# iris1997jiatong/I-DCCRN-VAE

Measured on AMD Instinct MI355X. Metric: 4s@16kHz utterances/sec fwd+SI-SNR, DCCRN-CL, 1/2/4/8 MI355X vs host CPU, higher is better.
Workload: dtype f32; 1 GPU; supervised DCCRN-CL forward(train=False) + final_ete_loss (weights 0/0/1); batch_per_gpu=64, utterance=4 s @ 16 kHz (64000 samples, 641 frames), parallelism=replicas x1, streams=1, input=resident in HBM

## Files before the change

### i-dccrn-vae_amd/csrc/ctconv_c1_f32.hip

```cpp
#include "cgemm.hpp"
#include "conv_epilogue.hpp"
#include "../../include/idccrn_hip.h"

namespace {

constexpr int C1F_NC = 4;
constexpr int C1F_PR = 4;

template <bool STATS>
__global__ __launch_bounds__(256) void ctconv_c1_f32_kernel(const CgemmArgs a, int rseg) {
    const int tid = threadIdx.x;
    const int m_lo = blockIdx.y * rseg;
    int m_hi = m_lo + rseg;
    if (m_hi > a.Fin) m_hi = a.Fin;
    int jcol[C1F_NC], c0[C1F_NC][2], c1[C1F_NC][2];
    bool inb[C1F_NC], keep[C1F_NC], cok[C1F_NC][2];
#pragma unroll
    for (int n = 0; n < C1F_NC; ++n) {
        const int j = (blockIdx.x * C1F_NC + n) * 256 + tid;
        jcol[n] = j;
        inb[n] = j < a.J;
#pragma unroll
        for (int h = 0; h < 2; ++h) {
            const int c = j + h + a.tshift;
            cok[n][h] = inb[n] && c >= 0 && c < a.J;
            c0[n][h] = cok[n][h] ? c : 0;
            const int b = c0[n][h] / a.Tp;
            c1[n][h] = (b / a.x1_div) * a.Tp + (c0[n][h] - b * a.Tp);
        }
        const int tp = j % a.Tp;
        keep[n] = inb[n] && tp >= 1 && tp <= a.t_valid;
    }
    const float slope = a.slope ? *a.slope : 1.0f;
    const bool has_act = a.slope != nullptr;
    const float bias0 = a.bias[0], bias1 = a.bias[1];
    const size_t plane0 = (size_t)a.Fin * a.Jp, plane1 = (size_t)a.Fin * a.Jp1;
    const int CC = 2 * (a.C0 + a.C1);

    float st[5] = {0.f, 0.f, 0.f, 0.f, 0.f};
    float pa[C1F_NC][10], pb[C1F_NC][10], pc[C1F_NC][10];
#pragma unroll
    for (int n = 0; n < C1F_NC; ++n)
#pragma unroll
        for (int i = 0; i < 10; ++i) pa[n][i] = pb[n][i] = pc[n][i] = 0.f;

    auto contract = [&](int m, float (&p)[C1F_NC][10]) {
#pragma unroll
        for (int n = 0; n < C1F_NC; ++n)
#pragma unroll
            for (int i = 0; i < 10; ++i) p[n][i] = 0.f;
        if (m < 0 || m >= a.Fin) return;
        for (int cc0 = 0; cc0 < CC; cc0 += C1F_PR) {
            float xv[C1F_PR][C1F_NC][2];
#pragma unroll
            for (int u = 0; u < C1F_PR; ++u) {
                const int cc = cc0 + u < CC ? cc0 + u : CC - 1;
                const int ci = cc >> 1, ri = cc & 1;
                const bool first = ci < a.C0;
                const float* r = first ? a.x0 + (size_t)(ri * a.C0 + ci) * plane0 + (size_t)m * a.Jp
                                       : a.x1 + (size_t)(ri * a.C1 + (ci - a.C0)) * plane1 + (size_t)m * a.Jp1;
#pragma unroll
                for (int n = 0; n < C1F_NC; ++n) {
                    xv[u][n][0] = r[first ? c0[n][0] : c1[n][0]];
                    xv[u][n][1] = r[first ? c0[n][1] : c1[n][1]];
                }
            }
#pragma unroll
            for (int u = 0; u < C1F_PR; ++u) {
                const bool live = cc0 + u < CC;
                const float* w = a.wfrag + (size_t)(live ? cc0 + u : 0) * 5 * 64;
#pragma unroll
                for (int kf = 0; kf < 5; ++kf) {
                    const float w00 = live ? w[kf * 64] : 0.f, w01 = live ? w[kf * 64 + 1] : 0.f;
                    const float w10 = live ? w[kf * 64 + 32] : 0.f, w11 = live ? w[kf * 64 + 33] : 0.f;
#pragma unroll
                    for (int n = 0; n < C1F_NC; ++n) {
                        const float x0v = cok[n][0] ? xv[u][n][0] : 0.f, x1v = cok[n][1] ? xv[u][n][1] : 0.f;
                        p[n][kf * 2] += w00 * x0v;
                        p[n][kf * 2 + 1] += w01 * x0v;
                        p[n][kf * 2] += w10 * x1v;
                        p[n][kf * 2 + 1] += w11 * x1v;
                    }
                }
            }
        }
    };
    auto emit = [&](int n, int fo, float yr, float yi) {
        if (fo < 0 || fo >= a.Fout) return;
        yr += bias0;
        yi += bias1;
        if (has_act) {
            yr = yr >= 0.f ? yr : slope * yr;
            yi = yi >= 0.f ? yi : slope * yi;
        }
        yr = keep[n] ? yr : 0.f;
        yi = keep[n] ? yi : 0.f;
        if (inb[n]) {
            a.out[(size_t)fo * a.Jp + jcol[n]] = yr;
            a.out[((size_t)a.Fout + fo) * a.Jp + jcol[n]] = yi;
        }
        if (STATS && keep[n]) epi_stats_add(st, yr, yi);
    };

    contract(m_lo - 1, pa);
    contract(m_lo, pb);
    for (int m = m_lo; m < m_hi; ++m) {
        contract(m + 1, pc);
#pragma unroll
        for (int n = 0; n < C1F_NC; ++n) {
            emit(n, 2 * m, pc[n][0] + pb[n][4] + pa[n][8], pc[n][1] + pb[n][5] + pa[n][9]);
            emit(n, 2 * m + 1, pc[n][2] + pb[n][6], pc[n][3] + pb[n][7]);
#pragma unroll
            for (int i = 0; i < 10; ++i) {
                pa[n][i] = pb[n][i];
                pb[n][i] = pc[n][i];
            }
        }
    }
    if (STATS) {
        __shared__ float red[4][5];
        const int lane = tid & 63, wave = tid >> 6;
#pragma unroll
        for (int s = 0; s < 5; ++s) {
            float t = st[s];
#pragma unroll
            for (int o = 32; o > 0; o >>= 1) t += __shfl_xor(t, o, 64);
            if (lane == 0) red[wave][s] = t;
        }
        __syncthreads();
        if (tid < 5) atomicAdd(&a.stats[tid], (double)red[0][tid] + (double)red[1][tid] + (double)red[2][tid] + (double)red[3][tid]);
    }
}

}

int idv_launch_ctconv_c1_f32(const CgemmArgs& a, hipStream_t st) {
    const int colblocks = (a.J + 256 * C1F_NC - 1) / (256 * C1F_NC);
    int segs = 512 / colblocks;
    if (segs < 1) segs = 1;
    if (segs > a.Fin) segs = a.Fin;
    const int rseg = (a.Fin + segs - 1) / segs;
    dim3 grid((unsigned)colblocks, (unsigned)((a.Fin + rseg - 1) / rseg));
    if (a.stats)
        hipLaunchKernelGGL(ctconv_c1_f32_kernel<true>, grid, dim3(256), 0, st, a, rseg);
    else
        hipLaunchKernelGGL(ctconv_c1_f32_kernel<false>, grid, dim3(256), 0, st, a, rseg);
    return idv_launch_status();
}
```

### include/idccrn_hip.h

```cpp
#ifndef IDCCRN_HIP_H
#define IDCCRN_HIP_H

#ifdef __cplusplus
extern "C" {
#endif

#define IDV_ABI_VERSION 9
#define IDV_SLACK_FLOATS 256

int idv_abi_version(void);

int idv_coop_last_status(int clear);
int idv_coop_max_workgroups(void);


int idv_cconv_cck(int cin_used);
int idv_cconv_config(int transposed, int cin_used, int Cout, int Fin);

int idv_cbn_fold(const float* moments, const float* gamma_rr, const float* gamma_ri, const float* gamma_ii,
                 const float* beta_r, const float* beta_i, int C, float* fold, void* stream);

int idv_pack_cconv(const float* w_re, const float* w_im, const float* b_re, const float* b_im, const float* fold,
                   int Cout, int Cin_total, int Cin_used, int transposed, float* wfrag, float* bias_out, void* stream);

int idv_pack_pw(const float* w, const float* bias, int M, int K, float* wfrag, float* bias_out, void* stream);

int idv_pack_lstm_ih(const float* w_ih_re, const float* b_ih_re, const float* b_hh_re, const float* w_ih_im,
                     const float* b_ih_im, const float* b_hh_im, int H, int K, float* wfrag, float* bias_out,
                     void* stream);
int idv_pack_lstm_hh(const float* w_hh_re, const float* w_hh_im, int H, float* whh_frag, void* stream);

int idv_make_dft(int n_fft, int win, int hop, int T, float* w_fwd, float* w_inv, float* env_inv, void* stream);


int idv_cconv2d_fwd(const float* x0, int C0, const float* x1, int C1, int Jp1, int x1_div, const float* wfrag,
                    const float* bias, const float* prelu_slope, float* out, double* stats, double* stats_work, int stats_rep,
                    int transposed, int tshift, int Cout, int Fin, int B, int Tp, int Jp, int t_valid_out, void* stream);

int idv_cconv_gauss_supported(int C0, int C1, int Cout);
long long idv_cconv_gauss_wfrag_floats(int Cout, int cin_used);
int idv_cconv_gauss_epi_rows(int Cout);
int idv_cconv_gauss_config(int transposed, int Cin, int Cout, int Fin);
int idv_pack_cconv_gauss(const float* w_re, const float* w_im, const float* b_re, const float* b_im, const float* fold, int Cout,
                         int Cin_total, int Cin_used, int transposed, int conj, float* wfrag, float* epi, void* stream);
int idv_cconv2d_gauss_fwd(const float* x0, int C0, const float* x1, int C1, int Jp1, int x1_div, const float* wfrag,
                          const float* epi, int has_fold, const float* prelu_slope, float* out, double* stats, double* stats_work,
                          int stats_rep, int transposed, int tshift, int Cout, int Fin, int B, int Tp, int Jp, int t_valid_out,
                          const float* addend, int addend_div, int addend_Jp, void* stream);

long long idv_cconv_bf16_wfrag_bytes(int Cout, int cin_used);
int idv_cconv_bf16_supported(int transposed, int C0, int C1, int x1_div, int Cout);
int idv_cconv_bf16_config(int transposed, int Cout, int Fin);
int idv_pack_cconv_bf16(const float* w_re, const float* w_im, const float* fold, int Cout, int Cin_total, int Cin_used,
                        int transposed, void* wfrag, void* stream);
int idv_cconv2d_bf16x3_fwd(const float* x0, int C0, const float* x1, int C1, int Jp1, int x1_div, const void* wfrag_bf16,
                           const float* bias, const float* prelu_slope, float* out, double* stats, double* stats_work,
                           int stats_rep, int transposed, int tshift, int Cout, int Fin, int B, int Tp, int Jp, int t_valid_out,
                           void* stream);

int idv_cconv2d_fwd_img(const float* x0, int C0, const float* x1, int C1, int Jp1, const float* wfrag, const float* bias,
                        const float* prelu_slope, float* out_planar, void* out_img, long long out_lo_off_elems,
                        int transposed, int tshift, int Cout, int Fin, int B, int Tp, int Jp, int t_valid_out,
                        void* stream);
int idv_cconv2d_img_train_fwd(const void* x0_img, long long lo_off0, int C0, const void* x1_img, long long lo_off1, int C1,
                              const void* wfrag_bf16, const float* bias, float* out_planar, double* stats, double* stats_work,
                              int stats_rep, int transposed, int Cout, int Fin, int B, int Tp, int Jp, int t_valid_out, void* stream);
int idv_cconv_img_config(int src_is_image, int transposed, int Cin, int Cout, int Fin);
int idv_planar_to_image(const float* x, int C, int F, int J, int Jp, void* img, long long lo_off_elems, void* stream);
int idv_planar_to_image_repeat(const float* x, int C, int F, int B, int Tp, int Jp_in, int rep, void* img, long long lo_off_elems,
                               int Jp, void* stream);
int idv_image_to_planar(const void* img, long long lo_off_elems, int C, int F, int J, int Jp, float* x, void* stream);
int idv_cconv2d_img_fwd(int src_is_image , const void* x0_img, long long lo_off0_slots, int C0, const void* x1_img, long long lo_off1_slots,
                        int C1, const void* wfrag_bf16, const float* bias, const float* prelu_slope, float* out_planar,
                        void* out_img, long long out_lo_off_elems, int transposed, int tshift,
                        int Cout, int Fin, int B, int Tp, int Jp, int t_valid_out, void* stream);

long long idv_ctconv_c1_wfrag_bytes(int cin_used);
int idv_pack_ctconv_c1_bf16(const float* w_re, const float* w_im, const float* fold, int Cin_total, int Cin_used,
                            void* wfrag, void* stream);
int idv_ctconv_c1_bf16x3_fwd(const float* x0, int C0, const float* x1, int C1, int Jp1, const void* wfrag,
                             const float* bias, const float* prelu_slope, float* out, int Fin, int B, int Tp, int Jp,
                             int t_valid_out, void* stream);
int idv_ctconv_c1_img_fwd(const void* x0_img, long long lo_off0_slots, int C0, const void* x1_img, long long lo_off1_slots,
                          int C1, const void* wfrag, const float* bias, const float* prelu_slope, float* out, int Fin, int B,
                          int Tp, int Jp, int t_valid_out, void* stream);

int idv_pw_gemm(const float* x, int K, const float* wfrag, const float* bias, const float* prelu_slope, float* out,
                int M, int B, int Tp, int Jp, int t_valid, int swap, int ldo, void* stream);
int idv_pw_gemm_form(int M, int swap, int Jp, const float* x);

int idv_cbn_finalize(const double* stats, double count, const float* gamma_rr, const float* gamma_ri,
                     const float* gamma_ii, const float* beta_r, const float* beta_i, int C, int first_call,
                     float momentum, float* running_mean_r, float* running_mean_i, float* Vrr, float* Vri,
                     float* Vii, float* moments, float* fold, void* stream);
int idv_cbn_stats(const float* act, int C, int F, int B, int Tp, int Jp, int t_valid, double* stats, void* stream);
int idv_cbn_apply_prelu(float* act, const float* fold, const float* prelu_slope, int C, int F, int B, int Tp, int Jp,
                        int t_valid, void* stream);

int idv_stft_frames(const float* x, int B, int L, int n_fft, int win, int hop, int T, float* frames, int Tp, int Jp,
                    void* stream);
int idv_istft_ola(const float* frames, const float* env_inv, int B, int n_fft, int win, int hop, int T, int Tp,
                  int Jp, float* y, void* stream);

int idv_mask_apply(const float* mask, const float* X, int x_div, int JpX, float* pred, float* pred_c, int F, int B,
                   int T, int Tp, int Jp, void* stream);
int idv_datanorm(const float* X, const float* mean, const float* stdv, int F, int B, int T, int Tp, int Jp, float* out, void* stream);
int idv_datadenorm(const float* P, const float* mean, const float* stdv, int F, int B, int T, int Tp, int Jp, float* out,
                   float* out_c, void* stream);
int idv_datanorm_bwd(const float* dout, const float* stdv, int F, int B, int T, int Tp, int Jp, float* dX, void* stream);
int idv_datadenorm_bwd(const float* dout, const float* dout_c, const float* stdv, int F, int B, int T, int Tp, int Jp, float* dP,
                       void* stream);
int idv_outtype_estimate(const float* speech_c, const float* noise_c, const float* X, long long sb, long long sf, long long st,
                         long long sr, int mode, int ns, int B, int F, int T, int Tp, int Jp, float* out, float* out_c,
                         void* stream);
int idv_planar_to_complex(const float* act, float* out_c, int F, int B, int T, int Tp, int Jp, void* stream);

long long idv_clstm_work_floats(int H, int B, int T, int Jp);
int idv_lstm_pers_supported(int H, int B);
long long idv_lstm_pers_work_bytes(int H, int B);
int idv_lstm_rec_pers(const float* g, long long g_run_z, long long g_run_s, int ldg, const float* whh_frag, float* hout, int H,
                      int B, int T, void* work, void* kimg, long long kimg_lo_slots, int Tp, int Jp, float* gsave, float* csave,
                      void* stream);
int idv_lstm_proj1_bf16x3(const void* himg, long long lo_off_slots, const void* wfrag_bf16, const float* bias, float* G1, int H,
                          int B, int T, int Tp, int Jp, void* stream);
int idv_lstm_coop_f32_supported(int H, int B);
long long idv_lstm_coop_f32_work_bytes(int H, int B);
int idv_lstm_rec_coop_f32(const float* g, long long g_run_z, long long g_run_s, int ldg, const float* whh_frag, float* hout, int H,
                          int B, int T, void* work, float* gsave, float* csave, void* stream);
int idv_lstm_pers_f32_supported(int H, int B);
long long idv_lstm_pers_f32_work_bytes(int H, int B);
int idv_lstm_rec_pers_f32(const float* g, long long g_run_z, long long g_run_s, int ldg, const float* whh_frag, float* hout, int H,
                          int B, int T, void* work, float* gsave, float* csave, void* stream);
void idv_lstm_pers_set_profile(unsigned long long* prof_cycles);
long long idv_clstm_train_work_floats(int H, int B, int T, int Jp);
int idv_clstm_fwd(const float* x, int K, const float* wih0, const float* bih0, const float* whh0, const float* wih1,
                  const float* bih1, const float* whh1, int H, int B, int T, int Tp, int Jp, float* work, float* out,
                  int flags, const void* wih1_bf16, void* stream);

int idv_lstm_stack2_f32_supported(int H, int B);
long long idv_lstm_stack2_f32_work_bytes(int H, int B);
int idv_lstm_stack2_f32(const float* g, long long g_run_z, long long g_run_s, int ldg, const float* whh0, const float* wih1_hh,
                        const float* whh1, const float* bias1, float* h0, float* hout, int H, int B, int T, void* work,
                        float* gsave1, float* csave0, float* csave1, void* stream);
int idv_clstm_fwd2(const float* x, int K, const float* wih0, const float* bih0, const float* whh0, const float* wih1,
                   const float* bih1, const float* whh1, const float* wih1_hh, int H, int B, int T, int Tp, int Jp, float* work,
                   float* out, int flags, const void* wih1_bf16, void* stream);

int idv_lstm_stack2_f32_proj_split(int H, int B, int T, int K, int force_c0, int* c0, int* P);
long long idv_lstm_stack2_f32_proj_work_bytes(int H, int B, int Tmax);
int idv_lstm_stack2_f32_proj(const float* x, int K, int Tp, int Jp, const float* wih0, const float* bih0, float* g,
                             const float* whh0, const float* wih1_hh, const float* whh1, const float* bias1, float* h0,
                             float* hout, int H, int B, int T, void* work, float* gsave1, float* csave0, float* csave1,
                             int force_c0, void* stream);
int idv_clstm_fwd3(const float* x, int K, const float* wih0, const float* bih0, const float* whh0, const float* wih1,
                   const float* bih1, const float* whh1, const float* wih1_hh, int H, int B, int T, int Tp, int Jp, float* work,
                   float* out, int flags, const void* wih1_bf16, int proj_c0, void* stream);

long long idv_lstm_ih_bf16_bytes(int H, int K);
int idv_lstm_proj_bf16_supported(int H, int K);
int idv_pack_lstm_ih_bf16(const float* w_ih_re, const float* w_ih_im, int H, int K, void* wfrag, void* stream);
int idv_planar_to_kimage(const float* x, int nvalid, int nplanes, int J, int Jp, void* img, long long lo_off_elems, void* stream);
int idv_pw_bf16_coltile(int M, int B, int Tp);
int idv_pw_bf16x3_rows(const void* ximg, long long lo_off_slots, int K, const void* wfrag_bf16, const float* bias, float* out_rows,
                       int M, int ldo, int B, int T, int Tp, int Jp, void* stream);
long long idv_pw_bf16_wfrag_bytes(int M, int K);
int idv_pack_pw_bf16(const float* w, int M, int K, void* wfrag, void* stream);
int idv_pw_bf16x3(const void* ximg, long long lo_off_slots, int K, const void* wfrag_bf16, const float* bias, float* out, int M,
                  int B, int Tp, int Jp, int t_valid, void* stream);
int idv_stft_frames_kimage(const float* x, int B, int L, int n_fft, int win, int hop, int T, void* img, long long lo_off_elems,
                           int Tp, int Jp, void* stream);
int idv_lstm_proj_bf16x3(const void* ximg, long long lo_off_slots, int K, const void* wfrag_bf16, const float* bias, float* G,
                         int H, int B, int T, int Tp, int Jp, void* stream);

int idv_reparam(const float* lat, int Hl, int off_miu, int off_ls, int off_dl, int zdim, const float* eps_r,
                const float* eps_i, int ns, int B, int T, int Tp, int Jp, float* z, int Jpz, void* stream);


int idv_sisnr(const float* source, int src_ld, int src_div, const float* est, int est_ld, int B, int L, double* work,
              float* out, void* stream);
int idv_sisdr(const float* ref, int ref_ld, const float* est, int est_ld, int B, int L, double* work, float* out, void* stream);
int idv_mean_over_samples(const float* x, int ns, int B, int L, float* out, void* stream);
int idv_recon_loss(const float* pred_c, const float* ori, long long sb, long long sf, long long st, long long sr,
                   int ori_div, int B, int F, int T, double* work, float* out, void* stream);
int idv_ckl(const float* q1, int H1, int Jp1, int o1_miu, int o1_ls, int o1_dl, const float* q2, int H2, int Jp2,
            int o2_miu, int o2_ls, int o2_dl, int zdim, float eps, int B, int T, int Tp, double* work, float* out,
            void* stream);
int idv_msd(const float* a, int Ca, int ca0, int JpA, const float* b, int Cb, int cb0, int JpB, int C, int F, int B, int Tp,
            int t_valid, double* work, float* out, void* stream);
long long idv_mi_work_floats(int B, int ns, int T, int zdim);
int idv_mi_fwd(const float* lat, int H, int Jp, int o_miu, int o_ls, int o_dl, const float* z, int Jpz, int zdim, int ns, int B,
               int T, int Tp, float eps, float* work, double* acc, float* out, void* stream);
int idv_mi_bwd(const float* lat, int H, int Jp, int o_miu, int o_ls, int o_dl, const float* z, int Jpz, int zdim, int ns, int B,
               int T, int Tp, float eps, const float* work, const float* gout, float* dlat, float* dz, void* stream);
int idv_miu_dist(const float* q1, int H1, int Jp1, int off1, const float* q2, int H2, int Jp2, int off2, int zdim,
                 int B, int T, int Tp, double* work, float* out, void* stream);


int idv_pack_cconv_adjoint(const float* w_re, const float* w_im, int Cout, int Cin_total, int Cin_used, int transposed,
                           float* wfrag, float* bias_out, void* stream);
int idv_pack_cconv_bf16_adjoint(const float* w_re, const float* w_im, int Cout, int Cin_total, int Cin_used, int transposed,
                                void* wfrag, void* stream);

long long idv_cconv_wgrad_work_floats(int Cs, int Cl, int B, int Tp);
int idv_cconv2d_bwd_weight(const float* x, int Cx, int ci_off, const float* dy, int Cout, int Cin_total, int transposed,
                           int tshift, int Fin, int B, int Tp, int Jp_x, int Jp_dy, float* work, long long work_floats,
                           float* dw_re, float* dw_im, void* stream);
long long idv_cconv_wgrad_bf16_work_floats(int Cs, int Cl, int B, int Tp);
int idv_cconv2d_bwd_weight_bf16x3(const float* x, int Cx, int ci_off, const float* dy, int Cout, int Cin_total, int transposed,
                                  int tshift, int Fin, int B, int Tp, int Jp_x, int Jp_dy, float* work, long long work_floats,
                                  float* dw_re, float* dw_im, void* stream);
int idv_cconv_wgrad_gauss_supported(int Cs, int Cl);
long long idv_cconv_wgrad_gauss_work_floats(int Cx, int Cout, int transposed, int Fin, int B, int Tp, int Jp_x, int Jp_dy);
int idv_cconv2d_bwd_weight_gauss(const float* x, int Cx, int ci_off, const float* dy, int Cout, int Cin_total, int transposed,
                                 int tshift, int Fin, int B, int Tp, int Jp_x, int Jp_dy, float* work, long long work_floats,
                                 float* dw_re, float* dw_im, void* stream);
int idv_cconv2d_bwd_bias(const double* stats_dy, int Cout, float* db_re, float* db_im, void* stream);

long long idv_pw_wgrad_work_floats(int M, int K, int J);
int idv_pw_bwd_weight(const float* dout, int M, int Jp_d, const float* x, int K, int Jp_x, int J, int shift, float* work,
                      long long work_floats, float* dw, int ldw, int rowmap, int H, int accumulate, void* stream);
int idv_pw_bwd_weight_bf16x3(const float* dout, int M, int Jp_d, const float* x, int K, int Jp_x, int J, int shift, float* work,
                             long long work_floats, float* dw, int ldw, int rowmap, int H, int accumulate, void* stream);
int idv_planar_rowsum(const float* x, int M, int Jp, int J, int accumulate, float* out, void* stream);

int idv_cbn_apply_prelu_to(const float* y, const float* fold, const float* prelu_slope, int C, int F, int B, int Tp, int Jp,
                           int t_valid, float* out, void* stream);
int idv_cbn_bwd_reduce(const float* dz, const float* y, const float* fold, const float* prelu_slope, int C, int F, int B,
                       int Tp, int Jp, int t_valid, double* sums, void* stream);
int idv_cbn_bwd_finalize(const double* sums, double count, const float* moments, const float* gamma_rr, const float* gamma_ri,
                         const float* gamma_ii, int C, float* coef, float* dgamma_rr, float* dgamma_ri, float* dgamma_ii,
                         float* dbeta_r, float* dbeta_i, float* dslope, float param_grad_scale, void* stream);
int idv_cbn_bwd_apply(const float* dz, const float* y, const float* fold, const float* coef, const float* prelu_slope, int C,
                      int F, int B, int Tp, int Jp, int t_valid, float* dy, void* stream);
int idv_cbn_apply_prelu_to_img(const float* y, const float* fold, const float* prelu_slope, int C, int F, int B, int Tp, int Jp,
                               int t_valid, float* out, void* img, long long lo_off_elems, void* stream);
int idv_cbn_bwd_apply_img(const float* dz, const float* y, const float* fold, const float* coef, const float* prelu_slope, int C,
                          int F, int B, int Tp, int Jp, int t_valid, float* dy, void* img, long long lo_off_elems, void* stream);

int idv_mask_apply_bwd(const float* mask, const float* X, int x_div, int JpX, const float* dpred, const float* dpred_c, int F,
                       int B, int T, int Tp, int Jp, float* dmask, float* dX, void* stream);
int idv_repeat_batch_bwd(const float* drep, int n, int rows, int B, int Tp, int Jp_rep, int Jp, float* dx, void* stream);
int idv_complex_to_planar(const float* in_c, float* act, int F, int B, int T, int Tp, int Jp, void* stream);
int idv_istft_ola_bwd(const float* dy, const float* env_inv, int B, int n_fft, int win, int hop, int T, int Tp, int Jp,
                      float* dframes, void* stream);
int idv_stft_frames_bwd(const float* dframes, int B, int L, int n_fft, int win, int hop, int T, int Tp, int Jp, float* dx,
                        void* stream);
int idv_reparam_bwd(const float* lat, int Hl, int off_miu, int off_ls, int off_dl, int zdim, const float* eps_r,
                    const float* eps_i, int ns, int B, int T, int Tp, int Jp, const float* dz, int Jpz, float* dlat, void* stream);

int idv_sisnr_bwd(const float* source, int src_ld, int src_div, const float* est, int est_ld, int B, int L, const double* work,
                  const float* grad_out, float* dest, void* stream);
int idv_recon_loss_bwd(const float* pred_c, const float* ori, long long sb, long long sf, long long st, long long sr,
                       int ori_div, int B, int F, int T, const float* g_cpx, const float* g_mag, float* dpred_c, void* stream);
int idv_ckl_bwd(const float* q1, int H1, int Jp1, int o1_miu, int o1_ls, int o1_dl, const float* q2, int H2, int Jp2,
                int o2_miu, int o2_ls, int o2_dl, int zdim, float eps, int B, int T, int Tp, const float* grad_out, float* dq1,
                void* stream);
int idv_miu_dist_bwd(const float* q1, int H1, int Jp1, int off1, const float* q2, int H2, int Jp2, int off2, int zdim, int B,
                     int T, int Tp, const float* grad_out, const float* loss_value, float* dq1, float* dq2, void* stream);

int idv_lstm_uncombine(const float* dout, int H, int B, int T, int Tp, int Jp, float* dh, void* stream);
int idv_pack_lstm_hh_bwd(const float* w_hh_re, const float* w_hh_im, int H, float* whhT, void* stream);
long long idv_lstm_bptt_work_floats(int H, int B);
int idv_lstm_bptt(float* gates, long long g_run_z, long long g_run_s, int ldg, const float* cstates, const float* dhout,
                  const float* whhT, int H, int B, int T, float* work, void* stream);
int idv_lstm_bptt_coop_supported(int H, int B);
int idv_lstm_bptt_stack2_supported(int H, int B);
long long idv_lstm_bptt_stack2_work_bytes(int H, int B);
int idv_lstm_bptt_stack2(float* g1, float* g0, long long g0_run_z, long long g0_run_s, int ldg0, const float* c1, const float* c0,
                         const float* dhout1, const float* whhT1, const float* wihT1, const float* whhT0, int H, int B, int T,
                         void* work, void* stream);
long long idv_lstm_bptt_coop_work_bytes(int H, int B);
int idv_lstm_bptt_coop(float* gates, long long g_run_z, long long g_run_s, int ldg, const float* cstates, const float* dhout,
                       const float* whhT, int H, int B, int T, void* work, void* stream);
int idv_rows_to_planar(const float* src, long long ld, int c0, int ncol, int B, int T, int Tp, int Jp, float* dst, void* stream);
int idv_lstm_bias_grad(const float* dGp, int H, int Jp, int J, int accumulate, float* db, void* stream);

int idv_bucket_gather(const long long* table, int n, long long total, float* flat, void* stream);
int idv_bucket_scatter(const long long* table, int n, long long total, const float* flat, float scale, void* stream);
int idv_bucket_adam(const long long* ptable, const long long* gtable, const float* gflat, float* exp_avg, float* exp_avg_sq,
                    int n, long long total, float lr, double beta1, double beta2, float eps, float weight_decay,
                    float bias_correction1, float bias_correction2_sqrt, float grad_scale, void* stream);

#define IDV_CLIP_RECORD_BYTES 32
#define IDV_CLIP_SUMSQ 0
#define IDV_CLIP_NORM 8
#define IDV_CLIP_COEF 16
#define IDV_CLIP_FINITE 20
#define IDV_CLIP_SKIPPED 24
int idv_bucket_sqnorm_partials(long long total);
int idv_bucket_sqnorm(const long long* ptable, const long long* gtable, const float* gflat, int n, long long total, float grad_scale,
                      double* partials, long long first, void* stream);
int idv_bucket_clip_finalize(const double* partials, int count, double max_norm, int guard, void* record, void* stream);
int idv_bucket_adam_clipped(const long long* ptable, const long long* gtable, const float* gflat, float* exp_avg, float* exp_avg_sq,
                            int n, long long total, float lr, double beta1, double beta2, float eps, float weight_decay,
                            float bias_correction1, float bias_correction2_sqrt, float grad_scale, const void* record, int guard,
                            long long t_host, void* stream);
int idv_bucket_scale(const long long* table, int n, long long total, const void* record, void* stream);

int idv_cconv_wino_supported(int transposed, int C0, int C1, int Cout, int Fin);
long long idv_cconv_wino_wfrag_floats(int transposed, int Cout, int cin_used);
int idv_cconv_wino_config(int transposed, int Cin, int Cout);
int idv_pack_cconv_wino(const float* w_re, const float* w_im, int Cout, int Cin_total, int Cin_used, int transposed, int conj,
                        float* wfrag, void* stream);
int idv_cconv2d_wino_fwd(const float* x0, int C0, const float* x1, int C1, const float* wfrag, const float* epi, int has_fold,
                         const float* prelu_slope, float* out, double* stats, double* stats_work, int stats_rep, int transposed,
                         int tshift, int Cout, int Fin, int B, int Tp, int Jp, int t_valid_out, const float* addend,
                         int addend_div, int addend_Jp, void* stream);

int idv_cconv_tw_supported(int C0, int C1, int Cout, int Fin);
long long idv_cconv_tw_wfrag_floats(int Cout, int cin_used);
int idv_pack_cconv_tw(const float* wino_frag, int Cout, int cin_used, float* tw_frag, void* stream);
int idv_ctconv2d_tw_fwd(const float* x0, int C0, const float* x1, int C1, const float* wfrag, const float* epi, int has_fold,
                        const float* prelu_slope, float* out, double* stats, double* stats_work, int stats_rep, int tshift,
                        int Cout, int Fin, int B, int Tp, int Jp, int t_valid_out, const float* addend, int addend_div,
                        int addend_Jp, void* stream);

int idv_cconv_tw2_supported(int Cin, int Cout, int Fin);
long long idv_cconv_tw2_wfrag_floats(int Cout, int cin_used);
int idv_pack_cconv_tw2(const float* wino_frag, int Cout, int cin_used, float* tw_frag, void* stream);
int idv_cconv2d_tw_fwd(const float* x0, int Cin, const float* wfrag, const float* epi, int has_fold, const float* prelu_slope,
                       float* out, double* stats, double* stats_work, int stats_rep, int tshift, int Cout, int Fin, int B, int Tp,
                       int Jp, int t_valid_out, void* stream);

long long idv_stream_cconv_wfloats(int Cin, int Cout);
int idv_stream_pack_cconv(const float* w_re, const float* w_im, const float* b_re, const float* b_im, int Cin, int Cout,
                          int transposed, float* w, float* bias, void* stream);
int idv_stream_cconv_splits(int transposed, int Cin, int Cout, int Fin, int B);
int idv_stream_cconv(const float* x0, const float* h0, int C0, const float* x1, const float* h1, int C1, const float* w,
                     const float* bias, const float* fold, const float* prelu_slope, float* out, float* hist_out, float* x0hist_out,
                     float* work, int nsplit, int transposed, int Cout, int Fin, int B, int k, int Tp, int Jp, void* stream);
int idv_stream_lstm_supported(int H);
int idv_stream_clstm(const float* G, const float* wt, const float* b1, float* state, float* hout, float* out, int H, int B, int k,
                     int Tp, int Jp, void* stream);
int idv_stream_frames(const float* ring, int R, const float* x, long long ldx, int n_new, long long n_prev, long long L_end, int B,
                      int n_fft, int win, int hop, long long t0, int k, float* frames, int Tp, int Jp, void* stream);
int idv_stream_ring(float* ring, int R, const float* x, long long ldx, int n_new, long long n_prev, int B, void* stream);
int idv_stream_ola(const float* frames, int Tp, int Jp, const float* carry_in, int carry_in_len, float* carry_out, int cap, int B,
                   int n_fft, int win, int hop, long long t0, int k, long long T_total, long long e0, long long e1, long long p_end,
                   float* y, int ldy, long long y_off, void* stream);

#define IDV_STREAM_ROW_FIELDS 12
#define IDV_ROW_N_PREV 0
#define IDV_ROW_COUNT 1
#define IDV_ROW_L_END 2
#define IDV_ROW_T0 3
#define IDV_ROW_K 4
#define IDV_ROW_PARITY 5
#define IDV_ROW_E0 6
#define IDV_ROW_E1 7
#define IDV_ROW_P_END 8
#define IDV_ROW_CARRY_IN 9
#define IDV_ROW_T_TOTAL 10
#define IDV_ROW_Y_OFF 11
int idv_stream_row_fields(void);
int idv_stream_rows_check(const long long* host_rows, int B, int R, int n_x, int n_fft, int win, int hop, int cap, int k_launch, int Tp,
                          long long ldy, long long span_max);
int idv_stream_frames_rows(const float* ring, int R, const float* x, long long ldx, const long long* rows, int B, int n_fft, int win,
                           int hop, int k_launch, float* frames, int Tp, int Jp, void* stream);
int idv_stream_ring_rows(float* ring, int R, const float* x, long long ldx, int n_x, const long long* rows, int B, void* stream);
int idv_stream_ola_rows(const float* frames, int Tp, int Jp, float* carry, int cap, const long long* rows, int B, int n_fft, int win,
                        int hop, int k_launch, long long span_max, float* y, long long ldy, void* stream);
int idv_stream_cconv_rows(const float* x0, const float* h0, int C0, const float* x1, const float* h1, int C1, const float* w,
                          const float* bias, const float* fold, const float* prelu_slope, float* out, float* hist, float* x0hist,
                          float* work, int nsplit, int transposed, int Cout, int Fin, int B, int k_launch, int Tp, int Jp,
                          const long long* rows, void* stream);
int idv_stream_clstm_rows(const float* G, const float* wt, const float* b1, float* state, float* hout, float* out, int H, int B,
                          int k_launch, int Tp, int Jp, const long long* rows, void* stream);
int idv_stream_zero_rows(float* buf, long long outer, int B, long long inner, const long long* slots, int n_slots, void* stream);

long long idv_stream_cconv_mfma_wfloats(int Cin, int Cout);
int idv_stream_pack_cconv_mfma(const float* w_re, const float* w_im, const float* b_re, const float* b_im, int Cin, int Cout,
                               int transposed, float* w, float* bias, void* stream);
int idv_stream_cconv_mfma_supported(int transposed, int Cin, int Cout);
int idv_stream_cconv_mfma(const float* x0, const float* h0, int C0, const float* x1, const float* h1, int C1, const float* w,
                          const float* bias, const float* fold, const float* prelu_slope, float* out, float* hist_out, float* x0hist_out,
                          float* work, int nsplit, int transposed, int Cout, int Fin, int B, int k, int Tp, int Jp, void* stream);
int idv_stream_cconv_mfma_rows(const float* x0, const float* h0, int C0, const float* x1, const float* h1, int C1, const float* w,
                               const float* bias, const float* fold, const float* prelu_slope, float* out, float* hist, float* x0hist,
                               float* work, int nsplit, int transposed, int Cout, int Fin, int B, int k_launch, int Tp, int Jp,
                               const long long* rows, void* stream);

int idv_stream_clstm_wide_supported(int H);
long long idv_stream_clstm_wide_hstep_floats(int H, int B, int k);
int idv_stream_clstm_wide(const float* G, const float* wt, const float* b1, float* state, float* hstep, float* out, int H, int B,
                          int k, int Tp, int Jp, void* stream);
int idv_stream_eps(long long seed, long long t0, int k, int B, int ns, int zdim, float* eps_r, float* eps_i, void* stream);
int idv_stream_repeat(const float* x, const float* hist, int C, int F, int B, int ns, int k, int Tp, int Jp, float* xn, float* histn,
                      int Jpn, void* stream);

int idv_stream_clstm_wide_rows(const float* G, const float* wt, const float* b1, float* state, float* hstep, float* out, int H, int B,
                               int k_launch, int Tp, int Jp, const long long* rows, void* stream);
int idv_stream_eps_rows(long long seed, const long long* rows, int B, int ns, int zdim, int k_launch, float* eps_r, float* eps_i,
                        void* stream);
int idv_stream_repeat_rows(const float* x, const float* hist, int C, int F, int B, int ns, int k_launch, int Tp, int Jp,
                           const long long* rows, float* xn, float* histn, int Jpn, void* stream);

int idv_stream_eps_pair(long long seed, long long t0, int k, int B, int ns, int zdim, float* eps_sr, float* eps_si, float* eps_nr,
                        float* eps_ni, void* stream);
int idv_stream_estimate(const float* speech, const float* noise, const float* X, int recon_mask, int mode, int ns, int F, int B,
                        int k, int Tp, int Jp, int Jpn, float* out, void* stream);

int idv_stream_eps_pair_rows(const long long* seeds, const long long* rows, int B, int ns, int zdim, int k_launch, float* eps_sr,
                             float* eps_si, float* eps_nr, float* eps_ni, void* stream);

#define IDV_STATE_MAX_VIEWS 64
#define IDV_STATE_VIEW_FIELDS 4
#define IDV_STATE_VIEW_ADDR 0
#define IDV_STATE_VIEW_OUTER 1
#define IDV_STATE_VIEW_INNER 2
#define IDV_STATE_VIEW_OFFSET 3
int idv_stream_state_check(const long long* views_host, int n_views, int B, const long long* slots_host, int n_slots,
                           long long per_slot);
int idv_stream_state_gather(const long long* views, int n_views, int B, const long long* slots, int n_slots, float* out,
                            long long per_slot, void* stream);
int idv_stream_state_scatter(const long long* views, int n_views, int B, const long long* slots, int n_slots, const float* in,
                             long long per_slot, void* stream);
int idv_stream_eps_pair_rows_as(const long long* seeds, const long long* draw_slots, const long long* rows, int B, int ns, int zdim,
                                int k_launch, float* eps_sr, float* eps_si, float* eps_nr, float* eps_ni, void* stream);

#define IDV_SR_TAPS_AUTO 0
#define IDV_SR_TAPS_MEM 1
#define IDV_SR_TAPS_LDS 2
int idv_stream_resample_hist(int up, int down);
long long idv_stream_resample_final(long long P, int up, int down);
int idv_stream_resample(float* hist, int H, int parity, const float* x, long long ldx, int n_new, long long P0, int flush, long long n0,
                        int m, int B, int up, int down, const float* taps, int taps_mode, float* y, long long ldy, void* stream);
#define IDV_SR_ROW_FIELDS 7
#define IDV_SR_ROW_P0 0
#define IDV_SR_ROW_COUNT 1
#define IDV_SR_ROW_N0 2
#define IDV_SR_ROW_M 3
#define IDV_SR_ROW_PARITY 4
#define IDV_SR_ROW_END 5
#define IDV_SR_ROW_IDLE 6
int idv_stream_resample_row_fields(void);
int idv_stream_resample_rows_check(const long long* host_rows, int B, int n_x, int up, int down, int H, long long ldy);
int idv_stream_resample_rows(float* hist, int H, const float* x, long long ldx, int n_x, const long long* rows, int B, int up, int down,
                             const float* taps, int taps_mode, float* y, long long ldy, void* stream);

int idv_stft_frames_ragged(const float* x, long long ldx, const int* lens, int B, int n_fft, int win, int hop, int Tmax, float* frames,
                           int Tp, int Jp, void* stream);
int idv_stft_frames_kimage_ragged(const float* x, long long ldx, const int* lens, int B, int n_fft, int win, int hop, int Tmax, void* img,
                                  long long lo_off_elems, int Tp, int Jp, void* stream);
int idv_istft_ola_ragged(const float* frames, const int* lens, int len_div, int B, int n_fft, int win, int hop, int Tmax, int Tp, int Jp,
                         float* y, long long ldy, void* stream);
int idv_sisdr_ragged(const float* ref, int ref_ld, const float* est, int est_ld, const int* lens, int B, double* work, float* out,
                     void* stream);

long long idv_stoi_work_bytes(int B, int Lmax, int fs);
int idv_stoi(const float* ref, long long ref_ld, const float* est, long long est_ld, const int* lens, int B, int Lmax, int fs,
             int extended, void* work, long long work_bytes, float* out, int* counts, void* stream);
int idv_rmse_ragged(const float* ref, long long ref_ld, const float* est, long long est_ld, const int* lens, int B, double* work,
                    float* out, void* stream);

int idv_resample_ntaps(int up, int down);
long long idv_resample_len(long long L, int up, int down);
int idv_resample(const float* x, long long ldx, const int* lens, int B, int L, int up, int down, const float* taps, float* y,
                 long long ldy, void* stream);
#define IDV_PAD_REFLECT 0
#define IDV_PAD_CONSTANT 1
int idv_stft_frames_ragged_pad(const float* x, long long ldx, const int* lens, int B, int n_fft, int win, int hop, int Tmax, int pad_mode,
                               float* frames, int Tp, int Jp, void* stream);
long long idv_spec_moments_work_bytes(int rows, int B, int Tp);
int idv_spec_moments_update(const float* spec, const int* lens, int B, int hop, int Tmax, int Tp, int Jp, int rows, double* state,
                            void* work, long long work_bytes, void* stream);
int idv_spec_moments_merge(double* state, const double* other, int rows, void* stream);

long long idv_trim_work_bytes(int B, int L, int hop);
int idv_trim_bounds(const float* x, long long ldx, const int* lens, int B, int L, int frame, int hop, double top_db, void* work,
                    long long work_bytes, int* bounds, double* power, long long ldp, void* stream);
int idv_trim_gather(const float* x, long long ldx, const int* bounds, int B, int Lout, float* y, long long ldy, void* stream);

int idv_latent_row_stats(const float* q, int H, int Jp, int Tp, int off_miu, int off_ls, int off_dl, int zdim, const int* frames, int B,
                         int T, double* work, double* out, void* stream);
int idv_latent_pair_dist(const float* qa, int Ha, int Jpa, int Tpa, int oa_miu, int oa_ls, int oa_dl, const float* qb, int Hb, int Jpb,
                         int Tpb, int ob_miu, int ob_ls, int ob_dl, int zdim, const int* frames, int B, int T, double* work, double* out,
                         void* stream);
int idv_miu_moments_chunk(void);
long long idv_miu_moments_work_bytes(int zdim, int B, int T);
int idv_miu_moments_update(const float* q, int H, int Jp, int Tp, int off_miu, int zdim, const int* frames, int B, int T, double* state,
                           void* work, long long work_bytes, void* stream);
int idv_miu_moments_merge(double* state, const double* other, int zdim, void* stream);
int idv_latent_set_moments(const float* x, int N, int D, double* mom, void* stream);
int idv_latent_silhouette(const float* x1, int N1, const float* x2, int N2, int D, const double* mom1, const double* mom2, double* work,
                          double* out, void* stream);

#define IDV_MIX_WIN_FIELDS 6
#define IDV_MIX_ROW_FIELDS 16
#define IDV_MIX_MAX_C 0
#define IDV_MIX_SUM_C2 1
#define IDV_MIX_MAX_V 2
#define IDV_MIX_SUM_V2 3
#define IDV_MIX_ACT_C2 4
#define IDV_MIX_ACT_V2 5
#define IDV_MIX_ACTIVE 6
#define IDV_MIX_A 7
#define IDV_MIX_B 8
#define IDV_MIX_SUM_Y2 9
#define IDV_MIX_MAX_Y 10
#define IDV_MIX_G_CLEAN 11
#define IDV_MIX_G_NOISE 12
#define IDV_MIX_LEVEL_DB 13
#define IDV_MIX_CLIPPED 14
#define IDV_MIX_LEN 15
long long idv_mix_work_bytes(int B, int L, int win);
int idv_mix_gains(const float* clean, const long long* clean_off, long long ldc, const float* noise, const long long* noise_off,
                  long long ldn, const int* lens, const int* noise_lens, const int* phase, int B, int L, int Ln, const double* par,
                  int segmental, double target_db, double clip, int win, double thresh_db, void* work, long long work_bytes, double* rows,
                  void* stream);
int idv_mix_write(const float* clean, const long long* clean_off, long long ldc, const float* noise, const long long* noise_off,
                  long long ldn, const int* lens, const int* noise_lens, const int* phase, int B, int L, int Ln, const double* rows,
                  float* noisy, float* clean_out, float* noise_out, long long ldy, void* stream);

int idv_reverb(const float* x, const long long* x_off, long long ldx, const float* h, const long long* h_off, long long ldh,
               const int* lens, const int* taps, const int* hist, int B, int L, int Kmax, float* y, long long ldy, void* stream);

#define IDV_TW_PAIR_T_EVEN 1
#define IDV_TW_PAIR_T_ODD 2
#define IDV_TW_PAIR_CONV 4
#define IDV_TW_PAIR_ALL 7
#define IDV_TW_PAIR_DEFAULT 7
int idv_tw_pair(int mask);
long long idv_tw_pair_launches(int reset);

long long idv_rlstm1_save_doubles(int B, int T);
long long idv_rlstm1_fwd_scratch_doubles(int K, int Jp);
long long idv_rlstm1_bwd_scratch_doubles(int K, int B, int Jp);
int idv_rlstm1_fwd(const float* x, int C, int F, int B, int T, int Tp, int Jp, const float* wih0, const float* whh0,
                   const float* bih0, const float* bhh0, const float* wih1, const float* whh1, const float* bih1,
                   const float* bhh1, double* save, double* scratch, float* y, void* stream);
int idv_rlstm1_bwd(const float* x, int C, int F, int B, int T, int Tp, int Jp, const float* dy, const float* wih0,
                   const float* whh0, const float* wih1, const float* whh1, const double* save, double* scratch,
                   float* dx, float* dwih0, float* dsmall, void* stream);
int idv_lsgan(const float* a, const float* b, long long n, float* out, void* stream);
int idv_lsgan_bwd(const float* a, const float* b, long long n, const float* gout, float* da, float* db, void* stream);

#define IDV_ASM_MAX_PIECES 64
#define IDV_ASM_MAX_TRIES 16
#define IDV_ASM_WIN_FIELDS 2
long long idv_asm_work_bytes(int R, int samples, int win);
int idv_asm_activity(const float* pool, long long pool_n, const long long* src, const int* len, const int* dst, const int* first,
                     const int* count, int npieces, const int* rowlen, int B, int tries, int samples, int win, double target_db,
                     double energy_thresh, double min_activity, void* work, long long work_bytes, double* rowstat, int* active,
                     int* windows, double* activity, int* chosen, int* accepted, void* stream);
int idv_asm_write(const float* pool, long long pool_n, const long long* src, const int* len, const int* dst, const int* first,
                  const int* count, int npieces, const int* chosen, int B, int tries, int samples, float* out, long long ldo,
                  void* stream);

int idv_conv3x3_tile(int which);
long long idv_conv3x3_wfloats(int Cin, int Cout);
int idv_conv3x3_pack(const float* w, int Cin, int Cout, float* packed, void* stream);
int idv_conv3x3_fwd(const float* x, const float* wp, const float* bias, int N, int H, int W, int Cin, int Cout, int pool, float* y,
                    void* stream);
int idv_conv3x3_c1_fwd(const float* f, const float* w1, const float* b1, int N, int H, int W, int C, float* y, void* stream);
int idv_conv3x3_c1_pool_fwd(const float* f, const float* w1, const float* b1, int N, int H, int W, int C, float* y, void* stream);
int idv_conv3x3_c1_fused_fwd(const float* f, const float* w1, const float* b1, int C1, const float* wp, const float* bias, int N, int H,
                             int W, int Cout, int pool, float* y, void* stream);
int idv_conv3x3_gmax(const float* x, int N, long long P, int C, float* out, void* stream);
long long idv_dnsmos_frontend_wfloats(void);
int idv_dnsmos_frontend_pack(const float* re, const float* im, float* packed, void* stream);
int idv_dnsmos_frontend(const float* x, long long ldx, const int* lengths, int B, const int* seg, int nseg, const float* mats,
                        float floor_p, float ln_div, float* feat, void* stream);
int idv_dnsmos_head(const float* g, int N, const float* w0, const float* b0, const float* w1, const float* b1, const float* w2,
                    const float* b2, float* raw, void* stream);
int idv_dnsmos_clip(const float* raw, int nseg, const int* first, const int* count, int B, const double* poly, double* out, void* stream);

long long idv_p808_mel_work_doubles(int nseg);
int idv_p808_mel(const float* x, long long ldx, const int* lengths, int B, const int* seg, int nseg, const double* dft, const double* mel,
                 double* S, double* smax, double* work, void* stream);
int idv_p808_db(const double* S, const double* smax, int nseg, long long per, float* feat, void* stream);
int idv_p808_head(const float* g, int N, const float* w0, const float* b0, const float* w1, const float* b1, const float* w2,
                  const float* b2, float* raw, void* stream);
int idv_p808_clip(const float* raw, int nseg, const int* first, const int* count, int B, double* out, void* stream);

#ifdef __cplusplus
}
#endif
#endif
```

Measured before the change: 1095 utterances/sec.

## Restructure transposed-conv C1 kernel into single-pass row sweep with pipelined loads

Rewrites the final complex transposed-conv kernel so each input row is contracted once, using carried partial sums instead of three rolling contraction buffers. Alternate row segments sweep in opposite directions. Input loads are double-buffered across channel rounds, and weights are read through the constant address space with a scheduling barrier. A mask-free fast path runs when all lanes are in bounds. Columns per thread drop from 4 to 2, and the grid is planned from an assumed resident count of 1024 with a runtime rseg override. Row segments now also recompute their halo rows, and the emit bounds are restricted so segments do not overlap. This trades extra halo contraction for fewer accumulator registers and better latency hiding.

Measured after the change: 1100 utterances/sec, median of 6. About the same (+0.4%).

```diff
diff --git a/i-dccrn-vae_amd/csrc/ctconv_c1_f32.hip b/i-dccrn-vae_amd/csrc/ctconv_c1_f32.hip
--- a/i-dccrn-vae_amd/csrc/ctconv_c1_f32.hip
+++ b/i-dccrn-vae_amd/csrc/ctconv_c1_f32.hip
@@ -1,32 +1,39 @@
+#include <atomic>
+#include <type_traits>
 #include "cgemm.hpp"
 #include "conv_epilogue.hpp"
+#include "ctconv_c1_plan.hpp"
 #include "../../include/idccrn_hip.h"
 
 namespace {
 
-constexpr int C1F_NC = 4;
 constexpr int C1F_PR = 4;
+constexpr int C1F_WAVES = 4;
+typedef __attribute__((address_space(4))) float C1fWeight;
 
 template <bool STATS>
-__global__ __launch_bounds__(256) void ctconv_c1_f32_kernel(const CgemmArgs a, int rseg) {
+__global__ __launch_bounds__(256, C1F_WAVES) void ctconv_c1_f32_kernel(const CgemmArgs a, int rseg) {
     const int tid = threadIdx.x;
-    const int m_lo = blockIdx.y * rseg;
-    int m_hi = m_lo + rseg;
-    if (m_hi > a.Fin) m_hi = a.Fin;
-    int jcol[C1F_NC], c0[C1F_NC][2], c1[C1F_NC][2];
+    int m_lo, m_hi;
+    c1_seg_rows(blockIdx.y, rseg, a.Fin, m_lo, m_hi);
+    int jcol[C1F_NC];
+    unsigned c0[C1F_NC][2], c1[C1F_NC][2];
     bool inb[C1F_NC], keep[C1F_NC], cok[C1F_NC][2];
+    bool lane_ok = true;
 #pragma unroll
     for (int n = 0; n < C1F_NC; ++n) {
-        const int j = (blockIdx.x * C1F_NC + n) * 256 + tid;
+        const int j = c1_col(blockIdx.x, n, tid);
         jcol[n] = j;
         inb[n] = j < a.J;
 #pragma unroll
         for (int h = 0; h < 2; ++h) {
             const int c = j + h + a.tshift;
             cok[n][h] = inb[n] && c >= 0 && c < a.J;
-            c0[n][h] = cok[n][h] ? c : 0;
-            const int b = c0[n][h] / a.Tp;
-            c1[n][h] = (b / a.x1_div) * a.Tp + (c0[n][h] - b * a.Tp);
+            lane_ok = lane_ok && cok[n][h];
+            const int cs = cok[n][h] ? c : 0;
+            const int b = cs / a.Tp;
+            c0[n][h] = 4u * (unsigned)cs;
+            c1[n][h] = 4u * (unsigned)((b / a.x1_div) * a.Tp + (cs - b * a.Tp));
         }
         const int tp = j % a.Tp;
         keep[n] = inb[n] && tp >= 1 && tp <= a.t_valid;
@@ -35,58 +42,16 @@
     const bool has_act = a.slope != nullptr;
     const float bias0 = a.bias[0], bias1 = a.bias[1];
     const size_t plane0 = (size_t)a.Fin * a.Jp, plane1 = (size_t)a.Fin * a.Jp1;
-    const int CC = 2 * (a.C0 + a.C1);
+    const int CC = 2 * (a.C0 + a.C1), CC0 = 2 * a.C0;
+    const int r_first = m_lo > 0 ? m_lo - 1 : 0, r_last = m_hi < a.Fin ? m_hi : a.Fin - 1;
+    const bool down = c1_seg_down(blockIdx.y);
+    const int m_start = down ? r_last : r_first, m_stop = down ? r_first - 1 : r_last + 1, m_step = down ? -1 : 1;
+    const int fo_lo = 2 * m_lo, fo_hi = 2 * m_hi - 1 < a.Fout ? 2 * m_hi - 1 : a.Fout - 1;
 
     float st[5] = {0.f, 0.f, 0.f, 0.f, 0.f};
-    float pa[C1F_NC][10], pb[C1F_NC][10], pc[C1F_NC][10];
-#pragma unroll
-    for (int n = 0; n < C1F_NC; ++n)
-#pragma unroll
-        for (int i = 0; i < 10; ++i) pa[n][i] = pb[n][i] = pc[n][i] = 0.f;
-
-    auto contract = [&](int m, float (&p)[C1F_NC][10]) {
-#pragma unroll
-        for (int n = 0; n < C1F_NC; ++n)
-#pragma unroll
-            for (int i = 0; i < 10; ++i) p[n][i] = 0.f;
-        if (m < 0 || m >= a.Fin) return;
-        for (int cc0 = 0; cc0 < CC; cc0 += C1F_PR) {
-            float xv[C1F_PR][C1F_NC][2];
-#pragma unroll
-            for (int u = 0; u < C1F_PR; ++u) {
-                const int cc = cc0 + u < CC ? cc0 + u : CC - 1;
-                const int ci = cc >> 1, ri = cc & 1;
-                const bool first = ci < a.C0;
-                const float* r = first ? a.x0 + (size_t)(ri * a.C0 + ci) * plane0 + (size_t)m * a.Jp
-                                       : a.x1 + (size_t)(ri * a.C1 + (ci - a.C0)) * plane1 + (size_t)m * a.Jp1;
-#pragma unroll
-                for (int n = 0; n < C1F_NC; ++n) {
-                    xv[u][n][0] = r[first ? c0[n][0] : c1[n][0]];
-                    xv[u][n][1] = r[first ? c0[n][1] : c1[n][1]];
-                }
-            }
-#pragma unroll
-            for (int u = 0; u < C1F_PR; ++u) {
-                const bool live = cc0 + u < CC;
-                const float* w = a.wfrag + (size_t)(live ? cc0 + u : 0) * 5 * 64;
-#pragma unroll
-                for (int kf = 0; kf < 5; ++kf) {
-                    const float w00 = live ? w[kf * 64] : 0.f, w01 = live ? w[kf * 64 + 1] : 0.f;
-                    const float w10 = live ? w[kf * 64 + 32] : 0.f, w11 = live ? w[kf * 64 + 33] : 0.f;
-#pragma unroll
-                    for (int n = 0; n < C1F_NC; ++n) {
-                        const float x0v = cok[n][0] ? xv[u][n][0] : 0.f, x1v = cok[n][1] ? xv[u][n][1] : 0.f;
-                        p[n][kf * 2] += w00 * x0v;
-                        p[n][kf * 2 + 1] += w01 * x0v;
-                        p[n][kf * 2] += w10 * x1v;
-                        p[n][kf * 2 + 1] += w11 * x1v;
-                    }
-                }
-            }
-        }
-    };
+
     auto emit = [&](int n, int fo, float yr, float yi) {
-        if (fo < 0 || fo >= a.Fout) return;
+        if (fo < fo_lo || fo > fo_hi) return;
         yr += bias0;
         yi += bias1;
         if (has_act) {
@@ -96,27 +61,148 @@
         yr = keep[n] ? yr : 0.f;
         yi = keep[n] ? yi : 0.f;
         if (inb[n]) {
-            a.out[(size_t)fo * a.Jp + jcol[n]] = yr;
-            a.out[((size_t)a.Fout + fo) * a.Jp + jcol[n]] = yi;
+            char* o = reinterpret_cast<char*>(a.out + (size_t)fo * a.Jp);
+            *reinterpret_cast<float*>(o + 4u * (unsigned)jcol[n]) = yr;
+            *reinterpret_cast<float*>(o + (size_t)a.Fout * a.Jp * 4 + 4u * (unsigned)jcol[n]) = yi;
         }
         if (STATS && keep[n]) epi_stats_add(st, yr, yi);
     };
 
-    contract(m_lo - 1, pa);
-    contract(m_lo, pb);
-    for (int m = m_lo; m < m_hi; ++m) {
-        contract(m + 1, pc);
+    auto run = [&](auto mask) {
+        constexpr bool MASK = decltype(mask)::value;
+        float acc[C1F_NC][10], car[C1F_NC][6];
 #pragma unroll
         for (int n = 0; n < C1F_NC; ++n) {
-            emit(n, 2 * m, pc[n][0] + pb[n][4] + pa[n][8], pc[n][1] + pb[n][5] + pa[n][9]);
-            emit(n, 2 * m + 1, pc[n][2] + pb[n][6], pc[n][3] + pb[n][7]);
-#pragma unroll
-            for (int i = 0; i < 10; ++i) {
-                pa[n][i] = pb[n][i];
-                pb[n][i] = pc[n][i];
-            }
-        }
-    }
+#pragma unroll
+            for (int i = 0; i < 10; ++i) acc[n][i] = 0.f;
+#pragma unroll
+            for (int i = 0; i < 6; ++i) car[n][i] = 0.f;
+        }
+        unsigned cx[C1F_NC][2];
+
+        auto round_end = [&](int cc0) {
+            const int lim = cc0 < CC0 ? CC0 : CC;
+            return cc0 + C1F_PR < lim ? cc0 + C1F_PR : lim;
+        };
+        auto load = [&](int m, int cc0, float (&xv)[C1F_PR][C1F_NC][2]) {
+            const bool first = cc0 < CC0;
+            if (cc0 == 0 || cc0 == CC0) {
+#pragma unroll
+                for (int n = 0; n < C1F_NC; ++n) {
+                    cx[n][0] = first ? c0[n][0] : c1[n][0];
+                    cx[n][1] = first ? c0[n][1] : c1[n][1];
+                }
+            }
+            const int last = round_end(cc0) - 1;
+            const int Cs = first ? a.C0 : a.C1, ci0 = first ? 0 : a.C0;
+            const size_t planes = first ? plane0 : plane1;
+            const float* xs = (first ? a.x0 : a.x1) + (size_t)m * (first ? a.Jp : a.Jp1);
+#pragma unroll
+            for (int n = 0; n < C1F_NC; ++n) {
+                asm volatile("" : "+v"(cx[n][0]));
+                asm volatile("" : "+v"(cx[n][1]));
+            }
+#pragma unroll
+            for (int u = 0; u < C1F_PR; ++u) {
+                const int cc = cc0 + u < last ? cc0 + u : last;
+                const int ci = cc >> 1, ri = cc & 1;
+                const char* r = reinterpret_cast<const char*>(xs + (size_t)(ri * Cs + ci - ci0) * planes);
+#pragma unroll
+                for (int n = 0; n < C1F_NC; ++n) {
+                    xv[u][n][0] = *reinterpret_cast<const float*>(r + cx[n][0]);
+                    xv[u][n][1] = *reinterpret_cast<const float*>(r + cx[n][1]);
+                }
+            }
+        };
+        auto plane_w = [&](int cc, float (&wv)[20]) {
+            const C1fWeight* w = (const C1fWeight*)(a.wfrag + (size_t)cc * 5 * 64 + (down ? 4 * 64 : 0));
+            const int ks = down ? -64 : 64;
+#pragma unroll
+            for (int kf = 0; kf < 5; ++kf) {
+                wv[kf * 4] = w[kf * ks];
+                wv[kf * 4 + 1] = w[kf * ks + 1];
+                wv[kf * 4 + 2] = w[kf * ks + 32];
+                wv[kf * 4 + 3] = w[kf * ks + 33];
+            }
+        };
+        auto plane_fma = [&](const float (&wv)[20], const float (&x)[C1F_NC][2]) {
+#pragma unroll
+            for (int kf = 0; kf < 5; ++kf)
+#pragma unroll
+                for (int n = 0; n < C1F_NC; ++n) {
+                    const float x0v = !MASK || cok[n][0] ? x[n][0] : 0.f, x1v = !MASK || cok[n][1] ? x[n][1] : 0.f;
+                    acc[n][kf * 2] += wv[kf * 4] * x0v;
+                    acc[n][kf * 2 + 1] += wv[kf * 4 + 1] * x0v;
+                    acc[n][kf * 2] += wv[kf * 4 + 2] * x1v;
+                    acc[n][kf * 2 + 1] += wv[kf * 4 + 3] * x1v;
+                }
+        };
+        auto fma = [&](int cc0, const float (&xv)[C1F_PR][C1F_NC][2]) {
+            const int end = round_end(cc0);
+            if (end - cc0 == C1F_PR) {
+                float wv[2][20];
+                plane_w(cc0, wv[0]);
+#pragma unroll
+                for (int u = 0; u < C1F_PR; ++u) {
+                    if (u + 1 < C1F_PR) plane_w(cc0 + u + 1, wv[(u + 1) & 1]);
+                    __builtin_amdgcn_sched_barrier(0);
+                    plane_fma(wv[u & 1], xv[u]);
+                    __builtin_amdgcn_sched_barrier(0);
+                }
+            } else {
+#pragma unroll
+                for (int u = 0; u < C1F_PR - 1; ++u)
+                    if (cc0 + u < end) {
+                        float wv[20];
+                        plane_w(cc0 + u, wv);
+                        plane_fma(wv, xv[u]);
+                    }
+            }
+        };
+        auto row_end = [&](int m) {
+#pragma unroll
+            for (int n = 0; n < C1F_NC; ++n) {
+                emit(n, 2 * m - 2 * m_step, car[n][0] + acc[n][0], car[n][1] + acc[n][1]);
+                emit(n, 2 * m - m_step, car[n][2] + acc[n][2], car[n][3] + acc[n][3]);
+                car[n][0] = car[n][4] + acc[n][4];
+                car[n][1] = car[n][5] + acc[n][5];
+#pragma unroll
+                for (int i = 2; i < 6; ++i) car[n][i] = acc[n][i + 4];
+#pragma unroll
+                for (int i = 0; i < 10; ++i) acc[n][i] = 0.f;
+            }
+        };
+
+        float xa[C1F_PR][C1F_NC][2], xb[C1F_PR][C1F_NC][2];
+        int m = m_start, cc0 = 0;
+        load(m, cc0, xa);
+        for (;;) {
+            int c2 = round_end(cc0), m2 = m;
+            if (c2 >= CC) { c2 = 0; m2 += m_step; }
+            bool more = m2 != m_stop;
+            load(more ? m2 : m, more ? c2 : cc0, xb);
+            fma(cc0, xa);
+            if (c2 == 0) row_end(m);
+            if (!more) break;
+            m = m2; cc0 = c2;
+            c2 = round_end(cc0);
+            if (c2 >= CC) { c2 = 0; m2 += m_step; }
+            more = m2 != m_stop;
+            load(more ? m2 : m, more ? c2 : cc0, xa);
+            fma(cc0, xb);
+            if (c2 == 0) row_end(m);
+            if (!more) break;
+            m = m2; cc0 = c2;
+        }
+#pragma unroll
+        for (int n = 0; n < C1F_NC; ++n) {
+            emit(n, 2 * m, car[n][0], car[n][1]);
+            emit(n, 2 * m + m_step, car[n][2], car[n][3]);
+        }
+    };
+    if (__all(lane_ok)) run(std::false_type{});
+    else run(std::true_type{});
+
     if (STATS) {
         __shared__ float red[4][5];
         const int lane = tid & 63, wave = tid >> 6;
@@ -132,18 +218,20 @@
     }
 }
 
+std::atomic<int> c1_force_rseg{0};
+
+}
+
+extern "C" int idv_ctconv_c1_rseg(int rseg) {
+    return rseg < 0 ? c1_force_rseg.load(std::memory_order_relaxed) : c1_force_rseg.exchange(rseg, std::memory_order_relaxed);
 }
 
 int idv_launch_ctconv_c1_f32(const CgemmArgs& a, hipStream_t st) {
-    const int colblocks = (a.J + 256 * C1F_NC - 1) / (256 * C1F_NC);
-    int segs = 512 / colblocks;
-    if (segs < 1) segs = 1;
-    if (segs > a.Fin) segs = a.Fin;
-    const int rseg = (a.Fin + segs - 1) / segs;
-    dim3 grid((unsigned)colblocks, (unsigned)((a.Fin + rseg - 1) / rseg));
+    const C1Plan p = c1_plan(a.J, a.Fin, 256 * C1F_WAVES, c1_force_rseg.load(std::memory_order_relaxed));
+    dim3 grid((unsigned)p.colblocks, (unsigned)p.segs);
     if (a.stats)
-        hipLaunchKernelGGL(ctconv_c1_f32_kernel<true>, grid, dim3(256), 0, st, a, rseg);
+        hipLaunchKernelGGL(ctconv_c1_f32_kernel<true>, grid, dim3(256), 0, st, a, p.rseg);
     else
-        hipLaunchKernelGGL(ctconv_c1_f32_kernel<false>, grid, dim3(256), 0, st, a, rseg);
+        hipLaunchKernelGGL(ctconv_c1_f32_kernel<false>, grid, dim3(256), 0, st, a, p.rseg);
     return idv_launch_status();
 }
diff --git a/i-dccrn-vae_amd/csrc/ctconv_c1_plan.hpp b/i-dccrn-vae_amd/csrc/ctconv_c1_plan.hpp
--- /dev/null
+++ b/i-dccrn-vae_amd/csrc/ctconv_c1_plan.hpp
@@ -0,0 +1,33 @@
+#pragma once
+#include <hip/hip_runtime.h>
+
+constexpr int C1F_NC = 2;
+constexpr int C1F_COLS = 256 * C1F_NC;
+
+struct C1Plan {
+    int colblocks;
+    int rseg;
+    int segs;
+    int one_round;
+};
+
+__host__ inline C1Plan c1_plan(int J, int Fin, int resident, int force_rseg) {
+    C1Plan p;
+    p.colblocks = (J + C1F_COLS - 1) / C1F_COLS;
+    int segs = resident / (p.colblocks > 0 ? p.colblocks : 1);
+    if (segs < 1) segs = 1;
+    if (segs > Fin) segs = Fin;
+    p.rseg = force_rseg > 0 ? (force_rseg < Fin ? force_rseg : Fin) : (Fin + segs - 1) / segs;
+    p.segs = (Fin + p.rseg - 1) / p.rseg;
+    p.one_round = (force_rseg <= 0 && p.colblocks <= resident) ? 1 : 0;
+    return p;
+}
+
+__host__ __device__ inline void c1_seg_rows(int seg, int rseg, int Fin, int& m_lo, int& m_hi) {
+    m_lo = seg * rseg;
+    m_hi = m_lo + rseg < Fin ? m_lo + rseg : Fin;
+}
+
+__host__ __device__ inline bool c1_seg_down(int seg) { return (seg & 1) != 0; }
+
+__host__ __device__ inline int c1_col(int cb, int n, int tid) { return (cb * C1F_NC + n) * 256 + tid; }
diff --git a/include/idccrn_hip.h b/include/idccrn_hip.h
--- a/include/idccrn_hip.h
+++ b/include/idccrn_hip.h
@@ -16,6 +16,7 @@
 
 int idv_cconv_cck(int cin_used);
 int idv_cconv_config(int transposed, int cin_used, int Cout, int Fin);
+int idv_ctconv_c1_rseg(int rseg);
 
 int idv_cbn_fold(const float* moments, const float* gamma_rr, const float* gamma_ri, const float* gamma_ii,
                  const float* beta_r, const float* beta_i, int C, float* fold, void* stream);
```
